# togatoga/kanpyo

Hardware: AMD Instinct MI355X
Metric: sentences/sec (higher is better)
Workload: dtype i32; 1 GPU; BASELINE configs[1] (cfg 2): 100k synthetic ~40-char sentences, batch 4096, IPADIC-shaped 392k-record dictionary; batch=4096, batches_in_flight=8, streams=3, long_streams=0, GPU_MAX_HW_QUEUES=4, residency=inputs resident in HBM, dense tokens left in HBM

## Files before the change

kanpyo_amd/csrc/kgpu_chartrie.cpp:

```cpp
#include <algorithm>
#include <cstdint>
#include <cstring>
#include <vector>

#include "kgpu_internal.h"

namespace kgpu {

namespace {

struct Edge { uint32_t parent; uint32_t cp; uint32_t child; };

struct ByteTrie {
    const std::vector<DaNode> &da;
    std::vector<uint32_t> start;
    std::vector<uint32_t> slot;
    explicit ByteTrie(const std::vector<DaNode> &d) : da(d) {
        const size_t n = da.size();
        start.assign(n + 1, 0);
        auto edge = [&](size_t q, uint32_t &p) -> bool {
            const int64_t pc = da[q].check;
            if (pc < 1 || (size_t)pc >= n || (size_t)pc == q) return false;
            const int64_t b = da[(size_t)pc].base;
            if (b < 0) return false;
// ... 69 lines not shown
    for (const Edge &e : edges) cps.push_back(e.cp);
    std::sort(cps.begin(), cps.end());
    cps.erase(std::unique(cps.begin(), cps.end()), cps.end());
    if (cps.size() >= 0xFFFFu) return false;
    auto code_of = [&](uint32_t cp) -> uint32_t {
        auto it = std::lower_bound(cps.begin(), cps.end(), cp);
        return (it != cps.end() && *it == cp) ? (uint32_t)(it - cps.begin()) + 1u : 0xFFFFu;
    };
    out.n_codes = (uint32_t)cps.size();

    std::vector<CtNode> &d2 = out.da;
    std::vector<uint32_t> nf;
    auto grow = [&](size_t need) {
        if (need <= d2.size()) return;
        const size_t n = std::max<size_t>(need, d2.size() * 2 + 1024), old = d2.size();
        d2.resize(n, CtNode{0, 0, 0, 0});
        nf.resize(n + 1);
        for (size_t q = old + 1; q <= n; ++q) nf[q] = (uint32_t)q;
    };
    nf.assign(1, 0u);
    grow((size_t)out.n_codes + 16);
    auto next_free = [&](uint32_t q) -> uint32_t {
        if (q >= d2.size()) grow((size_t)q + 1);
        uint32_t r = q;
        while (nf[r] != r) r = nf[r];
        for (uint32_t x = q; x != r;) { const uint32_t y = nf[x]; nf[x] = r; x = y; }
        if (r >= d2.size()) grow((size_t)r + 1);
        return r;
    };
    auto take = [&](uint32_t q) { nf[q] = q + 1; };
    take(0); take(1);
    std::vector<uint32_t> slot_of(n_nodes, 0);
    slot_of[0] = 1;
    d2[1] = CtNode{0, 0, 0, 0};
    uint32_t cursor = 2;
    std::vector<uint32_t> codes;
    for (uint32_t cn = 0; cn < n_nodes; ++cn) {
        const uint32_t e0 = first_edge[cn], e1 = first_edge[cn + 1];
        codes.clear();
        for (uint32_t e = e0; e < e1; ++e) codes.push_back(code_of(edges[e].cp));
        const uint32_t ps = slot_of[cn];
        d2[ps].leaf = leaf_of[cn];
        if (codes.empty()) continue;
        const uint32_t c0 = codes.front(), cmax = codes.back();
        uint32_t q = next_free(std::max(codes.size() > 1 ? cursor : 2u, c0 + 1));
        uint32_t tries = 0;
        for (;;) {
            const uint32_t b = q - c0;
            grow((size_t)b + cmax + 1);
            bool ok = true;
            for (size_t k = 1; k < codes.size() && ok; ++k) { const uint32_t t = b + codes[k]; ok = nf[t] == t; }
            if (ok) {
                d2[ps].base = (int32_t)b;
                size_t k = 0;
                for (uint32_t e = e0; e < e1; ++e, ++k) {
                    const uint32_t t = b + codes[k];
                    d2[t] = CtNode{0, (int32_t)ps, 0, 0};
                    take(t);
                    slot_of[edges[e].child] = t;
                }
                break;
            }
            if (++tries == 64 && codes.size() > 1) { cursor = q; }
            q = next_free(q + 1);
        }
        if (d2.size() > (1ull << 31) - 70000) return false;
    }
    size_t last = d2.size();
    while (last > 2 && d2[last - 1].check == 0) --last;
    d2.resize(last);

    out.rec.assign(65536, CharRec{0, 0, 0xFFFFu, 0, 0, 0});
    const int32_t rb = d2[1].base;
    for (uint32_t cp = 0; cp < 65536; ++cp) {
        CharRec &r = out.rec[cp];
        r.cat = cat_len ? (cp < cat_len ? cat[cp] : cat[0]) : 0;
        const uint32_t code = cp == 0xFFFFu ? 0xFFFFu : code_of(cp);
        r.code = (uint16_t)code;
        if (code != 0xFFFFu) {
            const uint64_t q = (uint64_t)(int64_t)rb + code;
            if (q < d2.size() && d2[(size_t)q].check == 1) { r.base = d2[(size_t)q].base; r.slot = (int32_t)q; r.leaf = d2[(size_t)q].leaf; }
        }
    }
    for (uint32_t cp : cps)
        if (cp >= 0xFFFFu) { out.nb_cp.push_back(cp); out.nb_code.push_back(code_of(cp)); }
    return true;
}

void build_key_table(const std::vector<DaNode> &da, const std::vector<std::pair<int64_t, uint64_t>> &dup, uint64_t n_morphs, std::vector<uint8_t> &bytes,
                     std::vector<uint64_t> &off) {
    bytes.clear();
    off.assign((size_t)n_morphs + 1, 0);
    if (da.size() < 2 || da[1].base < 0 || n_morphs == 0) return;
    const ByteTrie bt(da);
    std::vector<uint64_t> shares((size_t)n_morphs, 0);
    for (const auto &kv : dup)
        if (kv.first >= 1 && (uint64_t)kv.first <= n_morphs) shares[(size_t)kv.first - 1] = kv.second;
    std::vector<uint32_t> key_at((size_t)n_morphs, 0xFFFFFFFFu), key_len((size_t)n_morphs, 0);
    std::vector<uint8_t> pool, path;
    struct Frame { uint32_t node, next, end; };
    std::vector<Frame> stack{Frame{1u, bt.start[1], bt.start[2]}};
    std::vector<uint8_t> seen(da.size(), 0);
    seen[1] = 1;
    while (!stack.empty()) {
        Frame &f = stack.back();
        if (f.next == f.end) { stack.pop_back(); if (!path.empty()) path.pop_back(); continue; }
        const uint32_t q = bt.slot[f.next++];
        const uint32_t c = (uint32_t)((int64_t)q - da[f.node].base);
        if (c == 0) {
            if (da[q].base < 0) {
                const uint64_t id = (uint64_t)(-(int64_t)da[q].base);
                if (id >= 1 && id <= n_morphs && pool.size() + path.size() < 0xFFFFFFFFu) {
                    const uint64_t last = std::min<uint64_t>(n_morphs, id + shares[(size_t)id - 1]);
                    for (uint64_t k = id; k <= last; ++k)
                        if (key_at[(size_t)k - 1] == 0xFFFFFFFFu) { key_at[(size_t)k - 1] = (uint32_t)pool.size(); key_len[(size_t)k - 1] = (uint32_t)path.size(); }
                    pool.insert(pool.end(), path.begin(), path.end());
                }
            }
            continue;
        }
        if (seen[q] || da[q].base < 0) continue;
        seen[q] = 1;
        path.push_back((uint8_t)c);
        stack.push_back(Frame{q, bt.start[q], bt.start[q + 1]});
    }
    for (size_t k = 0; k < (size_t)n_morphs; ++k) {
        off[k] = bytes.size();
        if (key_at[k] != 0xFFFFFFFFu) bytes.insert(bytes.end(), pool.begin() + key_at[k], pool.begin() + key_at[k] + key_len[k]);
    }
    off[(size_t)n_morphs] = bytes.size();
}

}

extern "C" int kgpu_debug_chartrie_search(const uint8_t *index_blob, size_t blob_len, const uint8_t *utf8, const uint64_t *offsets, uint64_t nq,
                                          uint32_t *out, uint64_t cap_pairs, uint64_t *out_offsets, uint64_t *info) {
    using namespace kgpu;
    if (!index_blob || blob_len < 8 || !offsets || !out_offsets || !info) return KGPU_ERR_INVALID_ARG;
    uint64_t n = 0;
    for (int k = 0; k < 8; ++k) n |= (uint64_t)index_blob[k] << (8 * k);
    if (n > (blob_len - 8) / 8) return KGPU_ERR_BAD_DICT;
    std::vector<DaNode> da((size_t)n);
    for (size_t i = 0; i < (size_t)n; ++i) {
        uint32_t b = 0, c = 0;
        for (int k = 0; k < 4; ++k) { b |= (uint32_t)index_blob[8 + 8 * i + k] << (8 * k); c |= (uint32_t)index_blob[12 + 8 * i + k] << (8 * k); }
        da[i] = DaNode{(int32_t)b, (int32_t)c};
    }
    CharTrie ct;
    const bool ok = build_char_trie(da, nullptr, 0, ct);
    info[0] = ct.da.size(); info[1] = ct.n_codes; info[2] = ok ? 1 : 0;
    uint64_t np = 0;
    for (uint64_t s = 0; s < nq; ++s) {
        out_offsets[s] = np;
        if (!ok) continue;
        const uint8_t *t = utf8 + offsets[s];
        const uint64_t len = offsets[s + 1] - offsets[s];
        uint64_t k = 0;
        int32_t p = 0, bp = 0;
        auto next_code = [&](uint32_t &code) -> bool {
            if (k >= len) return false;
            const uint8_t b = t[k];
            const uint32_t l = b < 0x80 ? 1 : b < 0xE0 ? 2 : b < 0xF0 ? 3 : 4;
            if (k + l > len) return false;
            uint32_t cp = l == 1 ? b : l == 2 ? (b & 0x1Fu) : l == 3 ? (b & 0x0Fu) : (b & 0x07u);
            for (uint32_t j = 1; j < l; ++j) cp = (cp << 6) | (t[k + j] & 0x3Fu);
            k += l;
            if (cp < 0xFFFFu) code = ct.rec[cp].code;
            else {
                auto it = std::lower_bound(ct.nb_cp.begin(), ct.nb_cp.end(), cp);
                code = (it != ct.nb_cp.end() && *it == cp) ? ct.nb_code[(size_t)(it - ct.nb_cp.begin())] : 0xFFFFu;
            }
            return true;
        };
        uint32_t code = 0;
        if (!next_code(code) || code == 0xFFFFu) continue;
        {
            const uint64_t q = (uint64_t)(int64_t)ct.da[1].base + code;
            if (q >= ct.da.size() || ct.da[(size_t)q].check != 1) continue;
            p = (int32_t)q; bp = ct.da[(size_t)q].base;
        }
        for (;;) {
            if (ct.da[(size_t)p].leaf < 0) {
                if (np < cap_pairs) { out[2 * np] = (uint32_t)(-(int64_t)ct.da[(size_t)p].leaf); out[2 * np + 1] = (uint32_t)k; }
                ++np;
            }
            uint32_t c = 0xFFFFu;
            if (!next_code(c) || c == 0xFFFFu) break;
            const uint64_t q = (uint64_t)(uint32_t)bp + c;
            if (q >= ct.da.size() || ct.da[(size_t)q].check != p) break;
            p = (int32_t)q; bp = ct.da[(size_t)q].base;
        }
    }
    out_offsets[nq] = np;
    return np > cap_pairs ? KGPU_ERR_CAPACITY : KGPU_OK;
}

extern "C" int kgpu_debug_key_table(const uint8_t *index_blob, size_t blob_len, uint64_t n_morphs, uint8_t *keys, uint64_t keys_cap, uint64_t *keys_len,
                                    uint64_t *key_offsets) {
    using namespace kgpu;
    if (!index_blob || blob_len < 8 || !keys_len || !key_offsets) return KGPU_ERR_INVALID_ARG;
    uint64_t n = 0, m = 0;
    std::memcpy(&n, index_blob, 8);
    if (n > (blob_len - 8) / 8) return KGPU_ERR_BAD_DICT;
    std::vector<DaNode> da((size_t)n);
    if (n) std::memcpy(da.data(), index_blob + 8, (size_t)n * 8);
    size_t at = 8 + (size_t)n * 8;
    if (blob_len - at >= 8) { std::memcpy(&m, index_blob + at, 8); at += 8; }
    if (m > (blob_len - at) / 16) return KGPU_ERR_BAD_DICT;
    std::vector<std::pair<int64_t, uint64_t>> dup((size_t)m);
    for (auto &kv : dup) { std::memcpy(&kv.first, index_blob + at, 8); std::memcpy(&kv.second, index_blob + at + 8, 8); at += 16; }
    std::vector<uint8_t> bytes;
    std::vector<uint64_t> off;
    build_key_table(da, dup, n_morphs, bytes, off);
    std::memcpy(key_offsets, off.data(), off.size() * 8);
    *keys_len = bytes.size();
    if (bytes.size() > keys_cap) return KGPU_ERR_CAPACITY;
    if (!bytes.empty()) std::memcpy(keys, bytes.data(), bytes.size());
    return KGPU_OK;
}
```

kanpyo_amd/csrc/kgpu_device.h:

```cpp
#pragma once
#include <hip/hip_runtime.h>

#include "kgpu_internal.h"
#include "kgpu_tilepack.h"

namespace kgpu {
namespace dev {

constexpr uint32_t NONE = 0xFFFFFFFFu;
constexpr int32_t INF = 1 << 30;
constexpr uint32_t MAX_UNKNOWN_LEN = 1024;

__device__ __forceinline__ uint32_t bcast32(uint32_t v) { return __builtin_amdgcn_readfirstlane(v); }
__device__ __forceinline__ uint64_t bcast64(uint64_t v) {
    uint32_t lo = __builtin_amdgcn_readfirstlane((uint32_t)v);
    uint32_t hi = __builtin_amdgcn_readfirstlane((uint32_t)(v >> 32));
    return ((uint64_t)hi << 32) | lo;
}
template <int CTRL, int ROWS>
__device__ __forceinline__ uint32_t dpp_add(uint32_t v) {
    return v + (uint32_t)__builtin_amdgcn_update_dpp(0, (int)v, CTRL, ROWS, 0xF, false);
}
__device__ __forceinline__ uint32_t wave_incl_scan(uint32_t v, uint32_t ) {
    v = dpp_add<0x111, 0xF>(v);
// ... 155 lines not shown
        nstart += boundary;
        ++k;
    }
    return steps;
}

template <class FA, class FB>
__device__ __forceinline__ uint32_t da_walk_first2(const DictView &d, const uint8_t *text, uint32_t B,
                                                   bool onA, uint32_t cpA, uint32_t kbA, uint32_t knA, FA &&matchA,
                                                   bool onB, uint32_t cpB, uint32_t kbB, uint32_t knB, FB &&matchB) {
    struct W { int32_t p, bp; uint32_t k, nstart; bool live; };
    W a{0, 0, knA, 1, false}, b{0, 0, knB, 1, false};
    uint32_t steps = 0;
    DaNode fa{0, 0}, fb{0, 0};
    if (onA) fa = d.first[cpA];
    if (onB) fb = d.first[cpB];
    if (onA) { if (fa.base == 0) steps += (uint32_t)fa.check; else { a.p = fa.base; a.bp = fa.check; a.live = true; steps += knA - kbA; } }
    if (onB) { if (fb.base == 0) steps += (uint32_t)fb.check; else { b.p = fb.base; b.bp = fb.check; b.live = true; steps += knB - kbB; } }
    while (a.live || b.live) {
        const bool moreA = a.live && a.k < B, moreB = b.live && b.k < B;
        const uint32_t cA = moreA ? text[a.k] : 0u, cB = moreB ? text[b.k] : 0u;
        const bool bndA = !moreA || (cA & 0xC0) != 0x80, bndB = !moreB || (cB & 0xC0) != 0x80;
        const uint32_t qA = (uint32_t)(a.bp + (int32_t)cA), qB = (uint32_t)(b.bp + (int32_t)cB);
        const bool prA = a.live && bndA && (uint32_t)a.bp < d.da_len, prB = b.live && bndB && (uint32_t)b.bp < d.da_len;
        const bool nxA = moreA && qA < d.da_len, nxB = moreB && qB < d.da_len;
        DaNode tA{0, 0}, nA{0, 0}, tB{0, 0}, nB{0, 0};
        if (prA) tA = d.da[a.bp];
        if (nxA) nA = d.da[qA];
        if (prB) tB = d.da[b.bp];
        if (nxB) nB = d.da[qB];
        if (a.live) {
            if (prA && tA.check == a.p && tA.base < 0) { uint32_t id, dup; leaf_decode(d, tA.base, id, dup); matchA(id, a.nstart, dup); }
            if (!moreA) a.live = false;
            else {
                ++steps;
                if (!nxA || nA.check != a.p) a.live = false;
                else { a.p = (int32_t)qA; a.bp = nA.base; a.nstart += bndA; ++a.k; }
            }
        }
        if (b.live) {
            if (prB && tB.check == b.p && tB.base < 0) { uint32_t id, dup; leaf_decode(d, tB.base, id, dup); matchB(id, b.nstart, dup); }
            if (!moreB) b.live = false;
            else {
                ++steps;
                if (!nxB || nB.check != b.p) b.live = false;
                else { b.p = (int32_t)qB; b.bp = nB.base; b.nstart += bndB; ++b.k; }
            }
        }
    }
    return steps;
}

template <class CODE, class F>
__device__ __forceinline__ void ct_walk(const DictView &d, int32_t p, int32_t bp, int32_t leaf, CODE &&code_at, F &&on_match, uint32_t depth = 1) {
    if (p == 0) return;
    for (;;) {
        if (leaf < 0) { uint32_t id, dup; leaf_decode(d, leaf, id, dup); on_match(id, depth, dup); }
        const uint32_t c = code_at(depth);
        const uint32_t q = (uint32_t)bp + c;
        CtNode nx = d.da2[(c != 0xFFFFu && q < d.da2_len) ? q : 0u];
        asm volatile("" : "+v"(nx.base), "+v"(nx.check), "+v"(nx.leaf));
        if (nx.check != p) break;
        p = (int32_t)q;
        bp = nx.base;
        leaf = nx.leaf;
        ++depth;
    }
}
template <class CA, class FA, class CB, class FB>
__device__ __forceinline__ void ct_walk2(const DictView &d, bool onA, CA &&codeA, FA &&matchA, bool onB, CB &&codeB, FB &&matchB) {
    struct W { int32_t p, bp; uint32_t depth; bool live; };
    const int32_t rb = d.da2[1].base;
    W a{1, rb, 0, onA}, b{1, rb, 0, onB};
    while (a.live || b.live) {
        const uint32_t cA = a.live ? codeA(a.depth) : 0xFFFFu, cB = b.live ? codeB(b.depth) : 0xFFFFu;
        const uint32_t qA = (uint32_t)a.bp + cA, qB = (uint32_t)b.bp + cB;
        CtNode nA = d.da2[(cA != 0xFFFFu && qA < d.da2_len) ? qA : 0u];
        CtNode nB = d.da2[(cB != 0xFFFFu && qB < d.da2_len) ? qB : 0u];
        asm volatile("" : "+v"(nA.base), "+v"(nA.check), "+v"(nA.leaf), "+v"(nB.base), "+v"(nB.check), "+v"(nB.leaf));
        if (a.live) {
            if (nA.check != a.p) a.live = false;
            else {
                a.p = (int32_t)qA; a.bp = nA.base; ++a.depth;
                if (nA.leaf < 0) { uint32_t id, dup; leaf_decode(d, nA.leaf, id, dup); matchA(id, a.depth, dup); }
            }
        }
        if (b.live) {
            if (nB.check != b.p) b.live = false;
            else {
                b.p = (int32_t)qB; b.bp = nB.base; ++b.depth;
                if (nB.leaf < 0) { uint32_t id, dup; leaf_decode(d, nB.leaf, id, dup); matchB(id, b.depth, dup); }
            }
        }
    }
}
__device__ __forceinline__ uint32_t ct_code_nonbmp(const DictView &d, uint32_t cp) {
    uint32_t lo = 0, hi = d.n_nb;
    while (lo < hi) { const uint32_t mid = (lo + hi) >> 1; if (d.nb_cp[mid] < cp) lo = mid + 1; else hi = mid; }
    return (lo < d.n_nb && d.nb_cp[lo] == cp) ? d.nb_code[lo] : 0xFFFFu;
}
__device__ __forceinline__ uint32_t utf8_cp_at(const uint8_t *t) {
    const uint32_t b = t[0];
    if (b < 0x80) return b;
    if (b < 0xE0) return ((b & 0x1Fu) << 6) | (t[1] & 0x3Fu);
    if (b < 0xF0) return ((b & 0x0Fu) << 12) | ((t[1] & 0x3Fu) << 6) | (t[2] & 0x3Fu);
    return ((b & 0x07u) << 18) | ((t[1] & 0x3Fu) << 12) | ((t[2] & 0x3Fu) << 6) | (t[3] & 0x3Fu);
}

template <class BY>
__device__ __forceinline__ uint32_t utf8_decode_lead(uint32_t b, uint32_t k, uint32_t B, BY &&byte_at, uint32_t &cp, uint32_t &bad) {
    uint32_t l;
    if (b < 0x80) { l = 1; cp = b; }
    else if (b >= 0xC2 && b <= 0xDF) { l = 2; cp = b & 0x1F; }
    else if ((b & 0xF0) == 0xE0) { l = 3; cp = b & 0x0F; }
    else if (b >= 0xF0 && b <= 0xF4) { l = 4; cp = b & 0x07; }
    else { l = 1; cp = 0; bad = 1; }
    if (k + l > B) { bad = 1; l = 1; }
    for (uint32_t j = 1; j < l; ++j) {
        const uint32_t bb = byte_at(k + j);
        if ((bb & 0xC0) != 0x80) bad = 1;
        cp = (cp << 6) | (bb & 0x3F);
    }
    if (l == 3 && (cp < 0x800 || (cp >= 0xD800 && cp <= 0xDFFF))) bad = 1;
    if (l == 4 && (cp < 0x10000 || cp > 0x10FFFF)) bad = 1;
    return l;
}

#define KGPU_LDS(T) __attribute__((address_space(3))) T
template <class T> __device__ __forceinline__ T lds_ld(uint32_t addr) { return *(const KGPU_LDS(T) *)(uintptr_t)addr; }
template <class T> __device__ __forceinline__ void lds_st(uint32_t addr, T v) { *(KGPU_LDS(T) *)(uintptr_t)addr = v; }
__device__ __forceinline__ uint2 lds_ld2(uint32_t addr) { const uint64_t v = lds_ld<uint64_t>(addr); return make_uint2((uint32_t)v, (uint32_t)(v >> 32)); }

__device__ __forceinline__ void wave_sync() {
    __builtin_amdgcn_fence(__ATOMIC_ACQ_REL, "wavefront");
    __builtin_amdgcn_wave_barrier();
}

template <int CTRL>
__device__ __forceinline__ int32_t dpp_i32(int32_t x) { return __builtin_amdgcn_update_dpp(0, x, CTRL, 0xF, 0xF, true); }
template <uint32_t LG>
__device__ __forceinline__ int32_t group_min_i32(int32_t v) {
    if constexpr (LG >= 1) v = min(v, dpp_i32<0xB1>(v));
    if constexpr (LG >= 2) v = min(v, dpp_i32<0x4E>(v));
// ... 155 lines not shown
```

kanpyo_amd/csrc/kgpu_internal.h:

```cpp
#pragma once
#include <cstddef>
#include <cstdint>
#include <string>
#include <utility>
#include <vector>

#include "../../include/kanpyo_gpu.h"
#include "kgpu_normalize_core.h"
#include "kgpu_pack_core.h"
#include "kgpu_decode_core.h"

namespace kgpu {

void set_error(const char *fmt, ...) __attribute__((format(printf, 1, 2)));

struct alignas(8) DaNode {
    int32_t base, check;
};
struct alignas(8) Morph8 {
    int16_t left, right, cost;
    uint16_t dup;
};
struct alignas(16) CatInfo {
    uint32_t flags;
    int32_t unk_first;
    uint32_t unk_count;
    uint32_t pad;
};
enum : uint32_t { CAT_INVOKE = 1u, CAT_GROUP = 2u, CAT_HAS_UNK = 4u };
struct alignas(16) CtNode { int32_t base, check, leaf, pad; };
struct alignas(16) CharRec {
    int32_t base, slot;
    uint16_t code;
    uint8_t cat, pad;
    int32_t leaf;
};
struct CharTrie {
    std::vector<CtNode> da;
    std::vector<CharRec> rec;
    std::vector<uint32_t> nb_cp, nb_code;
    uint32_t n_codes = 0;
};
bool build_char_trie(const std::vector<DaNode> &da, const uint8_t *cat, size_t cat_len, CharTrie &out);
void build_key_table(const std::vector<DaNode> &da, const std::vector<std::pair<int64_t, uint64_t>> &dup, uint64_t n_morphs, std::vector<uint8_t> &bytes,
                     std::vector<uint64_t> &off);

struct DictView {
    const DaNode *da;        uint32_t da_len;
    uint32_t leaf_dup;
    const DaNode *first;
    const Morph8 *morph;     uint32_t n_morph;
    const Morph8 *unk_morph; uint32_t n_unk_morph;
    const int16_t *conn;     uint32_t conn_rows;
    uint32_t bos_right, eos_left;
    const uint8_t *cat;      uint32_t cat_len;
    const CatInfo *cinfo;
    const CtNode *da2;       uint32_t da2_len; uint32_t n_nb;
    const CharRec *crec;
    const uint32_t *nb_cp;   const uint32_t *nb_code;
};

struct Control {
    unsigned int ovf_count[4];
    unsigned int late_count[4];
    unsigned long long arena_cursor;
    unsigned int arena_overflow;
    unsigned int pad0;
    unsigned long long n_tokens;
    unsigned long long work[7];
    unsigned long long phase[10];
    unsigned int waves_done;
    unsigned int waves_copied;
    unsigned int small_flag;
    unsigned int pack_overflow;
    unsigned int window_fail;
    unsigned int small_abort;
    unsigned int win_ticket;
    unsigned int pad3;
    unsigned long long dump[8];
};

struct BatchArgs {
    const uint8_t *utf8;
    const uint64_t *offsets;
    uint64_t n;
    Control *ctl;
    uint8_t *arena;  uint64_t arena_bytes;
// ... 270 lines not shown
```

kanpyo_amd/csrc/kgpu_kernels.hip:

```cpp
#include <hip/hip_runtime.h>

#include <type_traits>

#include "kgpu_chain.h"
#include "kgpu_device.h"

namespace kgpu {

using namespace dev;

namespace {

constexpr uint32_t GMAXM = 8;

}

__global__ __launch_bounds__(64) void k_tokenize_general(DictView d, BatchArgs a, WorkIO io, uint32_t stop_after ) {
    const uint32_t lane = threadIdx.x;
    Slab sa{nullptr, 0}, sn{nullptr, 0};
    const int32_t base_root = d.da[1].base;
    uint64_t accW[7] = {0, 0, 0, 0, 0, 0, 0};

    for (uint32_t iter = 0;; ++iter) {
        uint64_t s = 0;
// ... 118 lines not shown
                uspan[i] = span;
                nb[i] = cnt;
            }
        }
        if (lane == 0) {
            nb[C] = 1;
            nb[C + 1] = 0;
            atomicAdd(&cnt_e[0], 1u);
        }
        __syncthreads();

#define KGPU_GSTOP(k) if (stop_after == (k)) { if (lane == 0) { a.status[s] = KGPU_SENT_TRUNCATED; a.tok_count[s] = 0; } continue; }
        KGPU_GSTOP(3)
        uint32_t ncarry = 1, bcarry = 0;
        for (uint32_t i0 = 0; i0 < C + 2; i0 += 64) {
            const uint32_t i = i0 + lane;
            const uint32_t v = i < C + 2 ? nb[i] : 0;
            const uint32_t w = i < C + 2 ? ld_l2(&boff[i]) : 0;
            const uint32_t vs = wave_incl_scan(v, lane), ws = wave_incl_scan(w, lane);
            if (i < C + 2) { nb[i] = ncarry + vs - v; boff[i] = bcarry + ws - w; }
            ncarry += __shfl(vs, 63, 64);
            bcarry += __shfl(ws, 63, 64);
        }
        const uint32_t N = bcast32(ncarry);
        __syncthreads();

        if (!(a.keep_lattice ? slab_fresh(sn, lat_scratch_off(N) + lat_scratch_bytes(N) + 64, a, lane) : slab_ensure(sn, (uint64_t)N * 44 + 64, a, lane))) {
            if (lane == 0) { a.status[s] = KGPU_SENT_NO_SCRATCH; a.tok_count[s] = 0; }
            continue;
        }
        uint4 *nodeA = (uint4 *)sn.ptr;
        uint4 *bucket = nodeA + N;
        uint2 *nodeB = (uint2 *)(bucket + N);
        uint32_t *pre = (uint32_t *)(nodeB + N);

        for (uint32_t i = lane; i < C; i += 64) {
            uint32_t t = nb[i];
            auto emit_match = [&](uint32_t id, uint32_t nch, uint32_t  = 0) {
                const uint32_t end = i + nch;
                const Morph8 m0 = d.morph[id - 1];
                const uint32_t nrec = 1u + m0.dup;
                for (uint32_t r = 0; r < nrec; ++r) {
                    const Morph8 m = r ? d.morph[id - 1 + r] : m0;
                    const uint32_t slot = boff[end] + atomicAdd(&fill_e[end], 1u);
                    nodeA[t] = make_uint4((uint16_t)m.left | ((uint32_t)(uint16_t)m.right << 16),
                                          (uint32_t)(int32_t)m.cost, slot, id + r);
                    nodeB[t] = make_uint2(i, end);
                    bucket[slot] = make_uint4((uint32_t)INF, (uint16_t)m.right, t, 0);
                    ++t;
                }
            };
            const uint32_t nm = mcnt[i];
            if (nm == 0xFFu) {
                if (ct) ct_walk(d, 1, d.da2[1].base, 0, [&](uint32_t dep) { return code_at(i + dep); }, emit_match, 0u);
                else da_walk(d, wtext, cbyte[i], B, base_root, emit_match);
            }
            else for (uint32_t m = 0; m < nm; ++m) emit_match(mid[(size_t)i * GMAXM + m], mnch[(size_t)i * GMAXM + m]);
            const uint32_t span = uspan[i];
            if (span) {
                const CatInfo ci = d.cinfo[ccat[i]];
                const uint32_t end = i + span;
                for (uint32_t r = 0; r < ci.unk_count; ++r) {
                    const Morph8 m = d.unk_morph[ci.unk_first - 1 + (int32_t)r];
                    const uint32_t slot = boff[end] + atomicAdd(&fill_e[end], 1u);
                    nodeA[t] = make_uint4((uint16_t)m.left | ((uint32_t)(uint16_t)m.right << 16),
                                          (uint32_t)(int32_t)m.cost, slot,
                                          (uint32_t)(-(ci.unk_first + (int32_t)r)));
                    nodeB[t] = make_uint2(i, end);
                    bucket[slot] = make_uint4((uint32_t)INF, (uint16_t)m.right, t, 0);
                    ++t;
                }
            }
        }
        if (lane == 0) {
            nodeA[N - 1] = make_uint4(d.eos_left, 0, NONE, 0);
            nodeB[N - 1] = make_uint2(C, C);
            bucket[0] = make_uint4(0, d.bos_right, 0, 0);
            pre[0] = NONE;
            if (a.keep_lattice) { nodeA[0] = make_uint4(d.bos_right << 16, 0, 0, 0); nodeB[0] = make_uint2(0, 0); }
        }
        __syncthreads();

        KGPU_GSTOP(5)
        auto global_step = [&](uint32_t q) {
            const uint32_t t0 = nb[q], t1 = nb[q + 1], p0 = boff[q], P = boff[q + 1] - p0;
            wE += (lane == 0) ? P * (t1 - t0) : 0;
            if (P >= 48) {
                for (uint32_t t = t0; t < t1; ++t) {
                    const uint4 na_ = nodeA[t];
                    const int16_t *col = d.conn + (size_t)d.conn_rows * (na_.x & 0xFFFFu);
                    int32_t best = 0x7FFFFFFF;
                    uint32_t bidx = NONE;
                    for (uint32_t j = lane; j < P; j += 64) {
                        const uint4 e = bucket[p0 + j];
                        const int32_t v = (int32_t)e.x + (int32_t)col[e.y];
                        if (v < best || (v == best && e.z < bidx)) { best = v; bidx = e.z; }
                    }
                    const int32_t vmin = wave_min_i32(best);
                    const uint32_t nmin = wave_min_u32(best == vmin ? bidx : NONE);
                    if (lane == 0) {
                        const int32_t tot = vmin + (int32_t)na_.y;
                        const bool ok = tot < INF;
                        pre[t] = ok ? nmin : NONE;
                        if (na_.z != NONE) bucket[na_.z].x = (uint32_t)(ok ? tot : INF);
                        else if (eos_dp) *eos_dp = (unsigned long long)(uint32_t)(ok ? tot : INF);
                    }
                }
// ... 386 lines not shown
```

kanpyo_amd/csrc/kgpu_pool.hip:

```cpp
#include <cstddef>
#include <cstdlib>
#include <type_traits>

#include "kgpu_device.h"
#include "kgpu_backtrace_core.h"

namespace kgpu {

using namespace dev;

namespace {

constexpr uint32_t MAXM = 8;
constexpr uint32_t NONE16 = 0xFFFFu;
#ifdef KGPU_ABSENT_TILES
constexpr bool ABSENT_TILES = true;
#else
constexpr bool ABSENT_TILES = false;
#endif
constexpr uint32_t DEAD_MARK = 1u << 16;
#ifndef KGPU_POOL_SLEEP
#define KGPU_POOL_SLEEP 16
#endif
#ifndef KGPU_EST_SLACK
// ... 232 lines not shown
        KGPU_STOP(1)
        KGPU_ARGS();

        uint32_t cb = 0, bad = 0, lensum = 0;
        for (uint32_t k0 = 0; k0 < B; k0 += 64) {
            const uint32_t k = k0 + lane;
            const uint32_t win = text_window(text, min(k, B));
            const bool start = (win & 0xC0u) != 0x80u;
            const uint64_t m = __ballot(start);
            const uint32_t ci = cb + __popcll(m & ((1ull << lane) - 1));
            uint32_t cp, bd = 0;
            const uint32_t l = utf8_decode_window(win, k, B, cp, bd);
            if (start) {
                bad |= bd;
                lensum += l;
                cbyte[ci] = (uint16_t)k;
                cp16[ci] = (uint16_t)(cp < 0xFFFFu ? cp : 0xFFFFu);
                if (cp >= 0xFFFFu) ccat[ci] = bad ? 0 : (cp < d.cat_len ? d.cat[cp] : d.cat[0]);
            }
            cb += __popcll(m);
        }
        lensum = bcast32(wave_sum(lensum));
        if (__ballot(bad != 0) != 0 || lensum != B) {
            if (lane == 0) { a.status[s] = KGPU_SENT_INVALID_UTF8; a.tok_count[s] = 0; }
            break;
        }
        if (lane == 0) cbyte[C] = (uint16_t)B;
        for (uint32_t e = lane; e < C + 2; e += 64) { boff[e] = 0; bfill[e] = 0; }
        wave_sync();

        KGPU_TICK(2);
        KGPU_STOP(2)
        KGPU_ARGS();
        uint32_t wT = 0, ovf = 0;
        {
            const int nchunks = (int)((C + 63) / 64);
            uint32_t carry_end = C;
            for (int ch = nchunks - 1; ch >= 0; --ch) {
                const uint32_t i = (uint32_t)ch * 64 + lane;
                const bool active = i < C;
                const uint32_t cpi = active ? cp16[i] : 0xFFFFu;
                uint32_t cat = 0x1FFu, ncat = 0x2FFu;
                uint32_t cnt = 0, m = 0;
                auto on_match = [&](uint32_t id, uint32_t nch, uint32_t dup) {
                    const uint32_t nrec = 1u + (dup != NONE ? dup : (uint32_t)d.morph[id - 1].dup);
                    if (m < MAXM && nch < 256) {
                        if (MS == 4) mbuf[i * MAXM + m] = id | (nch << 21) | ((nrec < 8 ? nrec : 0u) << 29);
                        else *(uint2 *)(mbuf + 2 * (i * MAXM + m)) = make_uint2(id, nch | (nrec << 8));
                    } else ovf = 1;
                    ++m;
                    cnt += nrec;
                    atomicAdd(&boff[i + nch], nrec);
                };
                if constexpr (!BYTE) {
                    const CharRec r = d.crec[cpi != 0xFFFFu ? cpi : 0u];
                    uint32_t code = 0xFFFFu;
                    int32_t p0 = 0, bp0 = 0, lf0 = 0;
                    if (active) {
                        if (cpi != 0xFFFFu) { cat = r.cat; code = r.code; p0 = r.slot; bp0 = r.base; lf0 = r.leaf; }
                        else {
                            cat = ccat[i];
                            code = d.n_nb ? ct_code_nonbmp(d, utf8_cp_at(text + cbyte[i])) : 0xFFFFu;
                            if (code != 0xFFFFu) {
                                const uint32_t q = (uint32_t)d.da2[1].base + code;
                                if (q < d.da2_len) { const CtNode nd = d.da2[q]; if (nd.check == 1) { p0 = (int32_t)q; bp0 = nd.base; lf0 = nd.leaf; } }
                            }
                        }
                        cp16[i] = (uint16_t)code;
                        ccat[i] = (uint8_t)cat;
                    }
                    wave_sync();
                    if (i + 1 < C) ncat = ccat[i + 1];
                    if (active) {
                        ct_walk(d, p0, bp0, lf0, [&](uint32_t dep) -> uint32_t { return i + dep < C ? (uint32_t)cp16[i + dep] : 0xFFFFu; }, on_match);
                        if constexpr (PROF) if (a.count_work == 1u) wT += da_walk_first(d, text, cpi, cbyte[i], cbyte[i + 1], B, base_root, [](uint32_t, uint32_t, uint32_t) {});
                        mcnt[i] = (uint8_t)(m < MAXM ? m : MAXM);
                    }
                } else {
                const uint32_t cpn = (i + 1 < C) ? cp16[i + 1] : 0u;
                if (active) cat = cpi != 0xFFFFu ? (cpi < d.cat_len ? d.cat[cpi] : d.cat[0]) : ccat[i];
                if (i + 1 < C) ncat = cpn != 0xFFFFu ? (cpn < d.cat_len ? d.cat[cpn] : d.cat[0]) : ccat[i + 1];
                if (active) {
                    wT += da_walk_first(d, text, cpi, cbyte[i], cbyte[i + 1], B, base_root, on_match);
                    mcnt[i] = (uint8_t)(m < MAXM ? m : MAXM);
                    ccat[i] = (uint8_t)cat;
                }
                }
                const uint64_t bm = __ballot(active && ncat != cat);
                const uint64_t rest = bm >> lane;
                const uint32_t run_end = rest ? i + (uint32_t)__ffsll((unsigned long long)rest) : carry_end;
                carry_end = bcast32(run_end);
                if (active) {
                    const CatInfo ci = d.cinfo[cat];
                    uint32_t span = 0;
                    if ((cnt == 0 || (ci.flags & CAT_INVOKE)) && (ci.flags & CAT_HAS_UNK) && ci.unk_count) {
                        span = 1;
                        if (ci.flags & CAT_GROUP) {
                            const uint32_t r = run_end - i;
                            span = r < MAX_UNKNOWN_LEN ? r : MAX_UNKNOWN_LEN;
                        }
                        cnt += ci.unk_count;
                        atomicAdd(&boff[i + span], ci.unk_count);
                        if (m < MAXM) {
                            if (MS == 4) mbuf[i * MAXM + m] = (uint32_t)ci.unk_first | ((ci.unk_count < 8 ? ci.unk_count : 0u) << 29);
                            else *(uint2 *)(mbuf + 2 * (i * MAXM + m)) = make_uint2((uint32_t)ci.unk_first, ci.unk_count);
                        }
                    }
                    uspan[i] = (uint16_t)span;
                    nb[i] = cnt;
                }
            }
        }
        if (__ballot(ovf != 0) != 0) { defer_s(s); break; }
        if (lane == 0) {
            nb[C] = 1;
            nb[C + 1] = 0;
            atomicAdd(&boff[0], 1u);
        }
        wave_sync();

        KGPU_TICK(3);
        KGPU_STOP(3)
        KGPU_ARGS();
        uint32_t ncarry = 1, bcarry = 0, tcarry = 0;
        uint64_t Esum = 0;
        for (uint32_t i0 = 0; i0 < C + 2; i0 += 64) {
            const uint32_t i = i0 + lane;
            const uint32_t v = i < C + 2 ? nb[i] : 0;
            const uint32_t w = i < C + 2 ? boff[i] : 0;
            const uint32_t x = ABSENT_TILES ? (v ? tile_groups(v) * max(1u, tile_groups(w)) : 0u) : tile_count(v, w);
            const uint32_t vs = wave_incl_scan(v, lane), ws = wave_incl_scan(w, lane), xs = wave_incl_scan(x, lane);
            if (i < C + 2) { nb[i] = ncarry + vs - v; boff[i] = bcarry + ws - w; ebase[i] = tcarry + xs - x; }
            ncarry += (uint32_t)__builtin_amdgcn_readlane((int)vs, 63);
            bcarry += (uint32_t)__builtin_amdgcn_readlane((int)ws, 63);
            tcarry += (uint32_t)__builtin_amdgcn_readlane((int)xs, 63);
            if constexpr (PROF) Esum += (uint64_t)v * w;
        }
        const uint32_t N = bcast32(ncarry), Nb = bcast32(bcarry), NT = bcast32(tcarry);

        off = align_up(off, 8);
        uint2 *node = (uint2 *)(smem + off);        off += 8 * (N + 1);
        int32_t *nSid = (int32_t *)(smem + off);    off += 4 * N;
        off = align_up(off, 8);
        const uint32_t off_emit_end = off;
        uint2 *bk = (uint2 *)(smem + off);          off += 8 * (Nb + (ABSENT_TILES ? 2 : 1));
        uint2 *tiles = (uint2 *)(smem + off);
// ... 339 lines not shown
```

kanpyo_amd/csrc/kgpu_window.hip:

```cpp
#include "kgpu_device.h"

namespace kgpu {

using namespace dev;

namespace {

#ifndef KGPU_WIN
#define KGPU_WIN 32
#endif
constexpr uint32_t WIN = KGPU_WIN;
static_assert(WIN >= 8 && WIN <= 63, "lane = position, and lane WIN holds the totals of the scans");
constexpr uint32_t REL = 2 * WIN + 1;
constexpr uint32_t NEARLEN = WIN;
constexpr uint32_t WMAXM = 8;
constexpr uint32_t XMAX = 48;
constexpr uint32_t LOOKB = 192;
constexpr uint32_t TEXTB = 4 * WIN + LOOKB;
constexpr uint32_t LCODE = 96;
constexpr uint32_t LTEXT = ((TEXTB + 4 > 260 ? TEXTB + 4 : 260) + 15) & ~15u;
static_assert(LTEXT / 4 <= 128, "two dwords per lane");
static_assert(2 * LCODE <= LTEXT && LCODE >= WIN && LCODE <= 128, "the codes share the text block's place");
constexpr uint32_t NCH_LOG = 13, NCHUNKS = 32;
constexpr uint32_t FCH_LOG = 12, FCHUNKS = 16;
// ... 376 lines not shown
            uint32_t fin = 0;
            uint32_t next_head_end = fhead_end;
            if (fhead < ftail && fhead_end < w0 + nw) {
                next_head_end = 0xFFFFFFFFu;
                for (uint32_t f0 = fhead; f0 < ftail; f0 += 64) {
                    const uint32_t f = f0 + lane;
                    bool in = false;
                    uint32_t e_end = 0xFFFFFFFFu;
                    if (f < ftail) { const Far e = *far_rec(f); e_end = e.end; in = e.end < w0 + nw; if (in) { atomicAdd(&fcnt[e.end - w0], 1u); if (e.node < rb) seed_bad = 1; } }
                    const uint64_t m = __ballot(in);
                    fin += __popcll(m);
                    if (m != ~0ull) {
                        next_head_end = (uint32_t)__builtin_amdgcn_readlane((int)e_end, (int)(__ffsll((unsigned long long)~m) - 1));
                        break;
                    }
                }
            }
            fin = bcast32(fin);
            if (__ballot(seed_bad != 0) != 0) { failed = true; why = 1; break; }
            wave_sync();
            {
                const uint32_t v = lane < nw ? fcnt[lane] : 0u;
                const uint32_t vs = wave_incl_scan(v, lane);
                if (lane < nw) {
                    fcnt[lane] = fhead + vs - v;
                    const bool wide = v >= WIDE_MIN;
                    wideN[lane] = wide ? v : 0u;
                    if (!wide && v) atomicAdd(&boff[lane], v);
                }
            }
            wave_sync();

            KW_T(2);
            KW_ARGS();
            uint32_t *mbuf = (uint32_t *)(lds + moff);
            uint32_t ovf = 0, cnt = 0, nfar = 0, wTw = 0, wEw = 0;
            if (lane < nwc) {
                uint32_t m = 0;
                auto on_match = [&](uint32_t id, uint32_t nch, uint32_t dup) {
                    const uint32_t nrec = 1u + (dup != NONE ? dup : (uint32_t)d.morph[id - 1].dup);
                    if (m < WMAXM && nch < 256) {
                        if (MS == 4) mbuf[lane * WMAXM + m] = id | (nch << 21) | ((nrec < 8 ? nrec : 0u) << 29);
                        else *(uint2 *)(mbuf + 2 * (lane * WMAXM + m)) = make_uint2(id, nch | (nrec << 8));
                    } else if (nch < 256 && m < 255 && nrec < 65536) {
                        const uint32_t k = atomicAdd(xcnt, 1u);
                        if (k < XMAX) xbuf[k] = make_uint2(lane | (nch << 8) | (nrec << 16), id); else ovf = 1;
                    } else ovf = 1;
                    ++m;
                    cnt += nrec;
                    if (nch <= NEARLEN) atomicAdd(&boff[lane + nch], nrec); else nfar += nrec;
                };
                if (ct) {
                    const uint16_t *lcode = (const uint16_t *)ltext;
                    ct_walk(d, 1, d.da2[1].base, 0, [&](uint32_t dep) -> uint32_t { const uint32_t j = lane + dep; return j < LCODE ? (uint32_t)lcode[j] : (uint32_t)code16[min(w0 + j, C)]; }, on_match, 0u);
                    if constexpr (PROF) if (!(a.count_work & 2u)) wTw += da_walk(d, text, cbw[lane], B, base_root, [](uint32_t, uint32_t, uint32_t) {});
                } else
                wTw += win_walk(d, byte, cp16w[lane], cbw[lane], cbw[lane + 1], B, base_root, on_match);
                mcnt[lane] = (uint8_t)m;
                const CatInfo ci = d.cinfo[catw[lane]];
                uint32_t span = 0;
                if ((cnt == 0 || (ci.flags & CAT_INVOKE)) && (ci.flags & CAT_HAS_UNK) && ci.unk_count) {
                    span = (ci.flags & CAT_GROUP) ? (uint32_t)rlenw[lane] : 1u;
                    cnt += ci.unk_count;
                    if (span <= NEARLEN) atomicAdd(&boff[lane + span], ci.unk_count); else nfar += ci.unk_count;
                    if (m < WMAXM) {
                        if (MS == 4) mbuf[lane * WMAXM + m] = (uint32_t)ci.unk_first | ((ci.unk_count < 8 ? ci.unk_count : 0u) << 29);
                        else *(uint2 *)(mbuf + 2 * (lane * WMAXM + m)) = make_uint2((uint32_t)ci.unk_first, ci.unk_count);
                    }
                }
                uspan[lane] = (uint16_t)span;
            } else if (lane < nw) { cnt = 1; mcnt[lane] = 0; uspan[lane] = 0; }
            if (__ballot(ovf != 0) != 0) { failed = true; why = 2; break; }
            wave_sync();

            KW_T(3);
            KW_ARGS();
            uint32_t N, Nb, NT, NF;
            {
                const uint32_t v = lane < nw ? cnt : 0u, fo = lane < nw ? nfar : 0u;
                const uint32_t vs = wave_incl_scan(v, lane), fs = wave_incl_scan(fo, lane);
                if (lane <= nw) { nb[lane] = vs - v; fbase[lane] = fs - fo; }
                N = (uint32_t)__builtin_amdgcn_readlane((int)vs, 63); NF = (uint32_t)__builtin_amdgcn_readlane((int)fs, 63);
                uint32_t bc = 0;
                for (uint32_t e0 = 0; e0 < REL + 1; e0 += 64) {
                    const uint32_t e = e0 + lane;
                    const uint32_t w = e < REL ? boff[e] : 0u;
                    const uint32_t ws = wave_incl_scan(w, lane);
                    if (e <= REL) boff[e] = bc + ws - w;
                    bc += (uint32_t)__builtin_amdgcn_readlane((int)ws, 63);
                }
                Nb = bc;
                wave_sync();
                const uint32_t P = lane < nw ? boff[lane + 1] - boff[lane] : 0u;
                const bool tiled = lane < nw && wideN[lane] == 0 && v != 0 && P != 0;
                const uint32_t x = tiled ? ((v + 7u) >> 3) * ((P + 7u) >> 3) : 0u;
                const uint32_t xs = wave_incl_scan(x, lane);
                if (lane <= nw) ebase[lane] = xs - x;
                NT = (uint32_t)__builtin_amdgcn_readlane((int)xs, 63);
                wEw = (lane < nw) ? v * (P + wideN[lane]) : 0u;
            }
            uint32_t off = off0;
            uint2 *bk = (uint2 *)(lds + off);            off += 8 * (Nb + NF + 1);
            uint8_t *brel = lds + off;                   off += align_up(Nb, 8);
            uint2 *node = (uint2 *)(lds + off);          off += 8 * (N + 1);
            int32_t *nSid = (int32_t *)(lds + off);      off += 4 * N;
            uint32_t *farEnd = (uint32_t *)(lds + off);  off += 4 * NF;
            uint16_t *nStart = (uint16_t *)(lds + off);  off += 2 * N;
// ... 489 lines not shown
```

Before: 158.9 million sentences/s.

## Add 32-bit child bitmask to char-trie nodes to skip failing transition loads

Each double-array char-trie node now stores a 32-bit bloom-style mask of its children's codes (bit = code mod 32) in the former pad word. The device walk checks this mask before issuing the dependent 16-byte node load and exits early when no child can match, which cuts global-memory round trips at the end of each walk. The CharRec slot field is replaced by a mask plus a has flag, with the root base pinned to a constant. The CatInfo load is also hoisted ahead of the wave sync so its latency overlaps the walk. The mask check adds a few ALU ops on every step, and the builder now fails for any layout where the root base is not the expected value.

```diff
diff --git a/kanpyo_amd/csrc/kgpu_chartrie.cpp b/kanpyo_amd/csrc/kgpu_chartrie.cpp
--- a/kanpyo_amd/csrc/kgpu_chartrie.cpp
+++ b/kanpyo_amd/csrc/kgpu_chartrie.cpp
@@ -145,6 +145,9 @@
             for (size_t k = 1; k < codes.size() && ok; ++k) { const uint32_t t = b + codes[k]; ok = nf[t] == t; }
             if (ok) {
                 d2[ps].base = (int32_t)b;
+                uint32_t mk = 0;
+                for (uint32_t c : codes) mk |= ct_child_bit(c);
+                d2[ps].mask = mk;
                 size_t k = 0;
                 for (uint32_t e = e0; e < e1; ++e, ++k) {
                     const uint32_t t = b + codes[k];
@@ -165,6 +168,7 @@
 
     out.rec.assign(65536, CharRec{0, 0, 0xFFFFu, 0, 0, 0});
     const int32_t rb = d2[1].base;
+    if (rb != CT_ROOT_BASE && rb != 0) return false;
     for (uint32_t cp = 0; cp < 65536; ++cp) {
         CharRec &r = out.rec[cp];
         r.cat = cat_len ? (cp < cat_len ? cat[cp] : cat[0]) : 0;
@@ -172,7 +176,7 @@
         r.code = (uint16_t)code;
         if (code != 0xFFFFu) {
             const uint64_t q = (uint64_t)(int64_t)rb + code;
-            if (q < d2.size() && d2[(size_t)q].check == 1) { r.base = d2[(size_t)q].base; r.slot = (int32_t)q; r.leaf = d2[(size_t)q].leaf; }
+            if (q < d2.size() && d2[(size_t)q].check == 1) { r.base = d2[(size_t)q].base; r.mask = d2[(size_t)q].mask; r.has = 1; r.leaf = d2[(size_t)q].leaf; }
         }
     }
     for (uint32_t cp : cps)
@@ -226,9 +230,10 @@
 
 }
 
-extern "C" int kgpu_debug_chartrie_search(const uint8_t *index_blob, size_t blob_len, const uint8_t *utf8, const uint64_t *offsets, uint64_t nq,
-                                          uint32_t *out, uint64_t cap_pairs, uint64_t *out_offsets, uint64_t *info) {
-    using namespace kgpu;
+namespace kgpu {
+namespace {
+int chartrie_search(const uint8_t *index_blob, size_t blob_len, const uint8_t *utf8, const uint64_t *offsets, uint64_t nq, uint32_t *out, uint64_t cap_pairs,
+                    uint64_t *out_offsets, uint64_t *info, uint64_t *out_loads, CharTrie *keep) {
     if (!index_blob || blob_len < 8 || !offsets || !out_offsets || !info) return KGPU_ERR_INVALID_ARG;
     uint64_t n = 0;
     for (int k = 0; k < 8; ++k) n |= (uint64_t)index_blob[k] << (8 * k);
@@ -245,11 +250,12 @@
     uint64_t np = 0;
     for (uint64_t s = 0; s < nq; ++s) {
         out_offsets[s] = np;
+        if (out_loads) out_loads[s] = 0;
         if (!ok) continue;
         const uint8_t *t = utf8 + offsets[s];
         const uint64_t len = offsets[s + 1] - offsets[s];
-        uint64_t k = 0;
-        int32_t p = 0, bp = 0;
+        uint64_t k = 0, loads = 0;
+        uint32_t first_cp = 0;
         auto next_code = [&](uint32_t &code) -> bool {
             if (k >= len) return false;
             const uint8_t b = t[k];
@@ -257,6 +263,7 @@
             if (k + l > len) return false;
             uint32_t cp = l == 1 ? b : l == 2 ? (b & 0x1Fu) : l == 3 ? (b & 0x0Fu) : (b & 0x07u);
             for (uint32_t j = 1; j < l; ++j) cp = (cp << 6) | (t[k + j] & 0x3Fu);
+            if (k == 0) first_cp = cp;
             k += l;
             if (cp < 0xFFFFu) code = ct.rec[cp].code;
             else {
@@ -265,27 +272,63 @@
             }
             return true;
         };
+        auto load = [&](uint64_t q) -> const CtNode & { ++loads; return ct.da[(size_t)q]; };
         uint32_t code = 0;
-        if (!next_code(code) || code == 0xFFFFu) continue;
-        {
-            const uint64_t q = (uint64_t)(int64_t)ct.da[1].base + code;
-            if (q >= ct.da.size() || ct.da[(size_t)q].check != 1) continue;
-            p = (int32_t)q; bp = ct.da[(size_t)q].base;
-        }
-        for (;;) {
-            if (ct.da[(size_t)p].leaf < 0) {
-                if (np < cap_pairs) { out[2 * np] = (uint32_t)(-(int64_t)ct.da[(size_t)p].leaf); out[2 * np + 1] = (uint32_t)k; }
+        int32_t p = 0, bp = 0, leaf = 0;
+        uint32_t mask = 0;
+        if (next_code(code) && code != CT_NO_CODE) {
+            if (first_cp < 0xFFFFu) {
+                const CharRec &r = ct.rec[first_cp];
+                if (r.has) { p = CT_ROOT_BASE + (int32_t)code; bp = r.base; leaf = r.leaf; mask = r.mask; }
+            } else {
+                const uint64_t q = (uint64_t)(uint32_t)ct.da[1].base + code;
+                if (q < ct.da.size()) { const CtNode &nd = load(q); if (nd.check == 1) { p = (int32_t)q; bp = nd.base; leaf = nd.leaf; mask = nd.mask; } }
+            }
+        }
+        while (p != 0) {
+            if (leaf < 0) {
+                if (np < cap_pairs) { out[2 * np] = (uint32_t)(-(int64_t)leaf); out[2 * np + 1] = (uint32_t)k; }
                 ++np;
             }
-            uint32_t c = 0xFFFFu;
-            if (!next_code(c) || c == 0xFFFFu) break;
+            uint32_t c = CT_NO_CODE;
+            if (!next_code(c)) c = CT_NO_CODE;
+            if (!ct_may_have_child(mask, c)) break;
             const uint64_t q = (uint64_t)(uint32_t)bp + c;
-            if (q >= ct.da.size() || ct.da[(size_t)q].check != p) break;
-            p = (int32_t)q; bp = ct.da[(size_t)q].base;
-        }
+            const CtNode &nx = load(q < ct.da.size() ? q : 0);
+            if (nx.check != p) break;
+            p = (int32_t)q; bp = nx.base; leaf = nx.leaf; mask = nx.mask;
+        }
+        if (out_loads) out_loads[s] = loads;
     }
     out_offsets[nq] = np;
+    if (keep) *keep = std::move(ct);
     return np > cap_pairs ? KGPU_ERR_CAPACITY : KGPU_OK;
+}
+}
+}
+
+extern "C" int kgpu_debug_chartrie_search(const uint8_t *index_blob, size_t blob_len, const uint8_t *utf8, const uint64_t *offsets, uint64_t nq,
+                                          uint32_t *out, uint64_t cap_pairs, uint64_t *out_offsets, uint64_t *info) {
+    return kgpu::chartrie_search(index_blob, blob_len, utf8, offsets, nq, out, cap_pairs, out_offsets, info, nullptr, nullptr);
+}
+extern "C" int kgpu_debug_chartrie_walk(const uint8_t *index_blob, size_t blob_len, const uint8_t *utf8, const uint64_t *offsets, uint64_t nq,
+                                        uint32_t *out, uint64_t cap_pairs, uint64_t *out_offsets, uint64_t *info, uint64_t *out_loads) {
+    if (!out_loads) return KGPU_ERR_INVALID_ARG;
+    return kgpu::chartrie_search(index_blob, blob_len, utf8, offsets, nq, out, cap_pairs, out_offsets, info, out_loads, nullptr);
+}
+extern "C" int kgpu_debug_chartrie_nodes(const uint8_t *index_blob, size_t blob_len, int32_t *nodes, uint64_t cap_nodes, uint32_t *recs, uint64_t *info) {
+    using namespace kgpu;
+    if (!nodes || !info) return KGPU_ERR_INVALID_ARG;
+    CharTrie ct;
+    const uint64_t offs[1] = {0};
+    uint64_t ooff[1] = {0};
+    const int rc = chartrie_search(index_blob, blob_len, nullptr, offs, 0, nullptr, 0, ooff, info, nullptr, &ct);
+    if (rc != KGPU_OK) return rc;
+    const size_t m = (size_t)std::min<uint64_t>(ct.da.size(), cap_nodes);
+    static_assert(sizeof(CtNode) == 16 && sizeof(CharRec) == 16, "one 16-byte load each");
+    if (m) std::memcpy(nodes, ct.da.data(), m * sizeof(CtNode));
+    if (recs && ct.rec.size() == 65536) std::memcpy(recs, ct.rec.data(), 65536 * sizeof(CharRec));
+    return KGPU_OK;
 }
 
 extern "C" int kgpu_debug_key_table(const uint8_t *index_blob, size_t blob_len, uint64_t n_morphs, uint8_t *keys, uint64_t keys_cap, uint64_t *keys_len,
diff --git a/kanpyo_amd/csrc/kgpu_ctmask.h b/kanpyo_amd/csrc/kgpu_ctmask.h
--- /dev/null
+++ b/kanpyo_amd/csrc/kgpu_ctmask.h
@@ -0,0 +1,17 @@
+#pragma once
+#include <cstdint>
+
+#if defined(__HIP__) || defined(__CUDACC__)
+#define KGPU_CT_HD __host__ __device__ inline __attribute__((always_inline))
+#else
+#define KGPU_CT_HD inline
+#endif
+
+namespace kgpu {
+
+constexpr uint32_t CT_NO_CODE = 0xFFFFu;
+
+KGPU_CT_HD constexpr uint32_t ct_child_bit(uint32_t code) { return 1u << (code & 31u); }
+KGPU_CT_HD constexpr bool ct_may_have_child(uint32_t mask, uint32_t code) { return code != CT_NO_CODE && (mask & ct_child_bit(code)) != 0; }
+
+}
diff --git a/kanpyo_amd/csrc/kgpu_device.h b/kanpyo_amd/csrc/kgpu_device.h
--- a/kanpyo_amd/csrc/kgpu_device.h
+++ b/kanpyo_amd/csrc/kgpu_device.h
@@ -231,43 +231,54 @@
 }
 
 template <class CODE, class F>
-__device__ __forceinline__ void ct_walk(const DictView &d, int32_t p, int32_t bp, int32_t leaf, CODE &&code_at, F &&on_match, uint32_t depth = 1) {
+__device__ __forceinline__ void ct_walk(const DictView &d, int32_t p, int32_t bp, int32_t leaf, uint32_t mask, CODE &&code_at, F &&on_match, uint32_t depth = 1) {
     if (p == 0) return;
     for (;;) {
         if (leaf < 0) { uint32_t id, dup; leaf_decode(d, leaf, id, dup); on_match(id, depth, dup); }
         const uint32_t c = code_at(depth);
+#ifndef KGPU_WALK_NO_MASK
+        if (!ct_may_have_child(mask, c)) break;
+#endif
         const uint32_t q = (uint32_t)bp + c;
+#ifndef KGPU_WALK_NO_MASK
+        CtNode nx = d.da2[q < d.da2_len ? q : 0u];
+#else
         CtNode nx = d.da2[(c != 0xFFFFu && q < d.da2_len) ? q : 0u];
-        asm volatile("" : "+v"(nx.base), "+v"(nx.check), "+v"(nx.leaf));
+#endif
+        asm volatile("" : "+v"(nx.base), "+v"(nx.check), "+v"(nx.leaf), "+v"(nx.mask));
         if (nx.check != p) break;
         p = (int32_t)q;
         bp = nx.base;
         leaf = nx.leaf;
+        mask = nx.mask;
         ++depth;
     }
 }
 template <class CA, class FA, class CB, class FB>
 __device__ __forceinline__ void ct_walk2(const DictView &d, bool onA, CA &&codeA, FA &&matchA, bool onB, CB &&codeB, FB &&matchB) {
-    struct W { int32_t p, bp; uint32_t depth; bool live; };
+    struct W { int32_t p, bp; uint32_t mask, depth; bool live; };
     const int32_t rb = d.da2[1].base;
-    W a{1, rb, 0, onA}, b{1, rb, 0, onB};
-    while (a.live || b.live) {
+    W a{1, rb, 0xFFFFFFFFu, 0, onA}, b{1, rb, 0xFFFFFFFFu, 0, onB};
+    for (;;) {
         const uint32_t cA = a.live ? codeA(a.depth) : 0xFFFFu, cB = b.live ? codeB(b.depth) : 0xFFFFu;
+        a.live = ct_may_have_child(a.mask, cA);
+        b.live = ct_may_have_child(b.mask, cB);
+        if (!(a.live || b.live)) break;
         const uint32_t qA = (uint32_t)a.bp + cA, qB = (uint32_t)b.bp + cB;
-        CtNode nA = d.da2[(cA != 0xFFFFu && qA < d.da2_len) ? qA : 0u];
-        CtNode nB = d.da2[(cB != 0xFFFFu && qB < d.da2_len) ? qB : 0u];
-        asm volatile("" : "+v"(nA.base), "+v"(nA.check), "+v"(nA.leaf), "+v"(nB.base), "+v"(nB.check), "+v"(nB.leaf));
+        CtNode nA = d.da2[(a.live && qA < d.da2_len) ? qA : 0u];
+        CtNode nB = d.da2[(b.live && qB < d.da2_len) ? qB : 0u];
+        asm volatile("" : "+v"(nA.base), "+v"(nA.check), "+v"(nA.leaf), "+v"(nA.mask), "+v"(nB.base), "+v"(nB.check), "+v"(nB.leaf), "+v"(nB.mask));
         if (a.live) {
             if (nA.check != a.p) a.live = false;
             else {
-                a.p = (int32_t)qA; a.bp = nA.base; ++a.depth;
+                a.p = (int32_t)qA; a.bp = nA.base; a.mask = nA.mask; ++a.depth;
                 if (nA.leaf < 0) { uint32_t id, dup; leaf_decode(d, nA.leaf, id, dup); matchA(id, a.depth, dup); }
             }
         }
         if (b.live) {
             if (nB.check != b.p) b.live = false;
             else {
-                b.p = (int32_t)qB; b.bp = nB.base; ++b.depth;
+                b.p = (int32_t)qB; b.bp = nB.base; b.mask = nB.mask; ++b.depth;
                 if (nB.leaf < 0) { uint32_t id, dup; leaf_decode(d, nB.leaf, id, dup); matchB(id, b.depth, dup); }
             }
         }
diff --git a/kanpyo_amd/csrc/kgpu_internal.h b/kanpyo_amd/csrc/kgpu_internal.h
--- a/kanpyo_amd/csrc/kgpu_internal.h
+++ b/kanpyo_amd/csrc/kgpu_internal.h
@@ -9,6 +9,7 @@
 #include "kgpu_normalize_core.h"
 #include "kgpu_pack_core.h"
 #include "kgpu_decode_core.h"
+#include "kgpu_ctmask.h"
 
 namespace kgpu {
 
@@ -28,11 +29,13 @@
     uint32_t pad;
 };
 enum : uint32_t { CAT_INVOKE = 1u, CAT_GROUP = 2u, CAT_HAS_UNK = 4u };
-struct alignas(16) CtNode { int32_t base, check, leaf, pad; };
+struct alignas(16) CtNode { int32_t base, check, leaf; uint32_t mask; };
+constexpr int32_t CT_ROOT_BASE = 1;
 struct alignas(16) CharRec {
-    int32_t base, slot;
+    int32_t base;
+    uint32_t mask;
     uint16_t code;
-    uint8_t cat, pad;
+    uint8_t cat, has;
     int32_t leaf;
 };
 struct CharTrie {
diff --git a/kanpyo_amd/csrc/kgpu_kernels.hip b/kanpyo_amd/csrc/kgpu_kernels.hip
--- a/kanpyo_amd/csrc/kgpu_kernels.hip
+++ b/kanpyo_amd/csrc/kgpu_kernels.hip
@@ -194,7 +194,7 @@
             };
             const uint32_t nm = mcnt[i];
             if (nm == 0xFFu) {
-                if (ct) ct_walk(d, 1, d.da2[1].base, 0, [&](uint32_t dep) { return code_at(i + dep); }, emit_match, 0u);
+                if (ct) ct_walk(d, 1, d.da2[1].base, 0, 0xFFFFFFFFu, [&](uint32_t dep) { return code_at(i + dep); }, emit_match, 0u);
                 else da_walk(d, wtext, cbyte[i], B, base_root, emit_match);
             }
             else for (uint32_t m = 0; m < nm; ++m) emit_match(mid[(size_t)i * GMAXM + m], mnch[(size_t)i * GMAXM + m]);
diff --git a/kanpyo_amd/csrc/kgpu_pool.hip b/kanpyo_amd/csrc/kgpu_pool.hip
--- a/kanpyo_amd/csrc/kgpu_pool.hip
+++ b/kanpyo_amd/csrc/kgpu_pool.hip
@@ -308,27 +308,32 @@
                     cnt += nrec;
                     atomicAdd(&boff[i + nch], nrec);
                 };
+                CatInfo ci = {0u, 0, 0u, 0u};
                 if constexpr (!BYTE) {
                     const CharRec r = d.crec[cpi != 0xFFFFu ? cpi : 0u];
                     uint32_t code = 0xFFFFu;
                     int32_t p0 = 0, bp0 = 0, lf0 = 0;
+                    uint32_t mk0 = 0;
                     if (active) {
-                        if (cpi != 0xFFFFu) { cat = r.cat; code = r.code; p0 = r.slot; bp0 = r.base; lf0 = r.leaf; }
+                        if (cpi != 0xFFFFu) { cat = r.cat; code = r.code; p0 = r.has ? CT_ROOT_BASE + (int32_t)r.code : 0; bp0 = r.base; lf0 = r.leaf; mk0 = r.mask; }
                         else {
                             cat = ccat[i];
                             code = d.n_nb ? ct_code_nonbmp(d, utf8_cp_at(text + cbyte[i])) : 0xFFFFu;
                             if (code != 0xFFFFu) {
                                 const uint32_t q = (uint32_t)d.da2[1].base + code;
-                                if (q < d.da2_len) { const CtNode nd = d.da2[q]; if (nd.check == 1) { p0 = (int32_t)q; bp0 = nd.base; lf0 = nd.leaf; } }
+                                if (q < d.da2_len) { const CtNode nd = d.da2[q]; if (nd.check == 1) { p0 = (int32_t)q; bp0 = nd.base; lf0 = nd.leaf; mk0 = nd.mask; } }
                             }
                         }
                         cp16[i] = (uint16_t)code;
                         ccat[i] = (uint8_t)cat;
                     }
+#ifndef KGPU_CATINFO_LATE
+                    ci = d.cinfo[cat & 0xFFu];
+#endif
                     wave_sync();
                     if (i + 1 < C) ncat = ccat[i + 1];
                     if (active) {
-                        ct_walk(d, p0, bp0, lf0, [&](uint32_t dep) -> uint32_t { return i + dep < C ? (uint32_t)cp16[i + dep] : 0xFFFFu; }, on_match);
+                        ct_walk(d, p0, bp0, lf0, mk0, [&](uint32_t dep) -> uint32_t { return i + dep < C ? (uint32_t)cp16[i + dep] : 0xFFFFu; }, on_match);
                         if constexpr (PROF) if (a.count_work == 1u) wT += da_walk_first(d, text, cpi, cbyte[i], cbyte[i + 1], B, base_root, [](uint32_t, uint32_t, uint32_t) {});
                         mcnt[i] = (uint8_t)(m < MAXM ? m : MAXM);
                     }
@@ -347,7 +352,10 @@
                 const uint32_t run_end = rest ? i + (uint32_t)__ffsll((unsigned long long)rest) : carry_end;
                 carry_end = bcast32(run_end);
                 if (active) {
-                    const CatInfo ci = d.cinfo[cat];
+#ifndef KGPU_CATINFO_LATE
+                    if constexpr (BYTE)
+#endif
+                    ci = d.cinfo[cat];
                     uint32_t span = 0;
                     if ((cnt == 0 || (ci.flags & CAT_INVOKE)) && (ci.flags & CAT_HAS_UNK) && ci.unk_count) {
                         span = 1;
diff --git a/kanpyo_amd/csrc/kgpu_window.hip b/kanpyo_amd/csrc/kgpu_window.hip
--- a/kanpyo_amd/csrc/kgpu_window.hip
+++ b/kanpyo_amd/csrc/kgpu_window.hip
@@ -452,7 +452,7 @@
                 };
                 if (ct) {
                     const uint16_t *lcode = (const uint16_t *)ltext;
-                    ct_walk(d, 1, d.da2[1].base, 0, [&](uint32_t dep) -> uint32_t { const uint32_t j = lane + dep; return j < LCODE ? (uint32_t)lcode[j] : (uint32_t)code16[min(w0 + j, C)]; }, on_match, 0u);
+                    ct_walk(d, 1, d.da2[1].base, 0, 0xFFFFFFFFu, [&](uint32_t dep) -> uint32_t { const uint32_t j = lane + dep; return j < LCODE ? (uint32_t)lcode[j] : (uint32_t)code16[min(w0 + j, C)]; }, on_match, 0u);
                     if constexpr (PROF) if (!(a.count_work & 2u)) wTw += da_walk(d, text, cbw[lane], B, base_root, [](uint32_t, uint32_t, uint32_t) {});
                 } else
                 wTw += win_walk(d, byte, cp16w[lane], cbw[lane], cbw[lane + 1], B, base_root, on_match);
```

Measured after the change: 160.3 million sentences/s, median of 4. Within noise of the previous version (+0.9%).
